# johnnypax/llm-kubernetes-minikube-sharp4dev

Hardware: AMD Instinct MI355X
Metric: RAG queries/sec (whole node) + p50 end-to-end latency, Llama-3-8B (higher is better)
Workload: dtype bf16

## Files before the change

### csrc/bindings.cpp

```cpp
#include <torch/extension.h>
#include <c10/hip/HIPStream.h>
#include "kernels.h"

namespace {

hipStream_t cur_stream() { return c10::hip::getCurrentHIPStream().stream(); }

#define CHECK_CUDA(x) TORCH_CHECK((x).is_cuda(), #x " must be a GPU tensor")
#define CHECK_BF16(x) TORCH_CHECK((x).scalar_type() == at::kBFloat16, #x " must be bfloat16")
#define CHECK_I32(x) TORCH_CHECK((x).scalar_type() == at::kInt, #x " must be int32")
#define CHECK_F32(x) TORCH_CHECK((x).scalar_type() == at::kFloat, #x " must be float32")
#define CHECK_LASTDIM(x) TORCH_CHECK((x).stride(-1) == 1, #x " must be contiguous in its last dim")
#define CHECK_CONTIG(x) TORCH_CHECK((x).is_contiguous(), #x " must be contiguous")
void check_rc(int rc, const char* name) {
  const hipError_t e = hipGetLastError();
  if (rc <= kLkAttrError && rc > kLkAttrError - 1000)
    TORCH_CHECK(false, name, ": kernel dynamic-LDS attribute refused: ", hipGetErrorString((hipError_t)(kLkAttrError - rc)));
  if (rc <= kLkLaunchError && rc > kLkLaunchError - 1000)
    TORCH_CHECK(false, name, ": kernel launch failed: ", hipGetErrorString((hipError_t)(kLkLaunchError - rc)));
  TORCH_CHECK(rc == 0, name, ": unsupported shape/config (code ", rc, ")");
  TORCH_CHECK(e == hipSuccess, name, ": kernel launch failed: ", hipGetErrorString(e));
}
#define CHECK_RC(rc, name) check_rc((rc), (name))

// ... 113 lines not shown
}

at::Tensor ws_linear(const at::Tensor& x, const at::Tensor& w, bool swiglu, int64_t bn, int64_t splits,
                     const c10::optional<at::Tensor>& out_) {
  CHECK_CUDA(x); CHECK_BF16(x); CHECK_BF16(w); CHECK_LASTDIM(x); CHECK_CONTIG(w);
  TORCH_CHECK(x.dim() == 2 && w.dim() == 2 && x.size(1) == w.size(1), "x [M,K], w [N,K]");
  check_rows16(x, "x"); check_rows16(w, "w");
  const int M = x.size(0), K = x.size(1), N = w.size(0);
  TORCH_CHECK(M >= 1 && M <= 256, "ws_linear: M must be in [1, 256]");
  const int n_out = swiglu ? N / 2 : N;
  at::Tensor out = out_ ? *out_ : at::empty({M, n_out}, x.options());
  CHECK_BF16(out); CHECK_LASTDIM(out);
  TORCH_CHECK(out.size(0) == M && out.size(1) == n_out, "out shape");
  int BN = (int)bn, S = (int)splits;
  if (BN <= 0 || S <= 0) {
    int pb = 64, ps = 1;
    lk_wsgemm_plan(M, N, K, swiglu ? 1 : 0, &pb, &ps);
    if (BN <= 0) BN = pb;
    if (S <= 0) S = ps;
  }
  at::Tensor part;
  if (S > 1) part = at::empty({(long)S * M * N}, x.options().dtype(at::kFloat));
  int rc = lk_wsgemm(bp(x), x.stride(0), bp(w), M, N, K, BN, S, swiglu ? 1 : 0, bp(out), out.stride(0),
                     S > 1 ? part.data_ptr<float>() : nullptr, cur_stream());
  CHECK_RC(rc, "ws_linear");
  return out;
}

namespace {
struct WsSplit {
  int M, N, K, BN, S;
};
WsSplit ws_split(const at::Tensor& x, const at::Tensor& w, int64_t bn, int64_t splits, const char* name) {
  CHECK_CUDA(x); CHECK_BF16(x); CHECK_BF16(w); CHECK_LASTDIM(x); CHECK_CONTIG(w);
  TORCH_CHECK(x.dim() == 2 && w.dim() == 2 && x.size(1) == w.size(1), name, ": x [M,K], w [N,K]");
  check_rows16(x, "x"); check_rows16(w, "w");
  WsSplit p{(int)x.size(0), (int)w.size(0), (int)x.size(1), (int)bn, (int)splits};
  TORCH_CHECK(p.M >= 1 && p.M <= 256, name, ": M must be in [1, 256]");
  if (p.BN <= 0 || p.S <= 0) {
    int pb = 64, ps = 1;
    lk_wsgemm_plan(p.M, p.N, p.K, 0, &pb, &ps);
    if (p.BN <= 0) p.BN = pb;
    if (p.S <= 0) p.S = ps;
  }
  TORCH_CHECK(p.S >= 2, name, ": needs a split-K plan (S >= 2)");
  return p;
}
}

at::Tensor ws_linear_rmsnorm(const at::Tensor& x, const at::Tensor& w, at::Tensor& residual,
                             const at::Tensor& norm_w, double eps, int64_t bn, int64_t splits,
                             const c10::optional<at::Tensor>& tickets) {
  const WsSplit p = ws_split(x, w, bn, splits, "ws_linear_rmsnorm");
  CHECK_CUDA(residual); CHECK_BF16(residual); CHECK_LASTDIM(residual); check_rows16(residual, "residual");
  TORCH_CHECK(residual.dim() == 2 && residual.size(0) == p.M && residual.size(1) == p.N, "residual shape");
  CHECK_BF16(norm_w); TORCH_CHECK(norm_w.numel() == p.N && norm_w.is_contiguous(), "norm weight shape");
// ... 353 lines not shown
  CHECK_RC(lk_gather_rows(bp(out), bp(x), x.stride(0), idx.data_ptr<int64_t>(), idx.numel(), x.size(1), cur_stream()),
           "gather_rows");
  return out;
}

int64_t gemm_streamk(int64_t mode) { return lk_gemm_streamk((int)mode); }

bool gemm_supported(int64_t M, int64_t N, int64_t K, int64_t epi, int64_t bn, int64_t splits, int64_t variant) {
  return gemm_shape_ok((int)M, (int)N, (int)K, (int)epi, (int)bn, (int)splits, (int)variant);
}

std::vector<int64_t> ws_plan(int64_t M, int64_t N, int64_t K, bool swiglu) {
  int bn = 64, s = 1;
  lk_wsgemm_plan((int)M, (int)N, (int)K, swiglu ? 1 : 0, &bn, &s);
  return {bn, s};
}

int64_t skinny_splits(int64_t M, int64_t N, int64_t K, bool swiglu) {
  return lk_skinny_splits((int)M, (int)N, (int)K, swiglu ? 1 : 0);
}

void activation_(at::Tensor& x, const c10::optional<at::Tensor>& bias, int64_t kind) {
  CHECK_CUDA(x); CHECK_BF16(x); CHECK_LASTDIM(x);
  TORCH_CHECK(x.dim() == 2, "x must be 2-D");
  check_rows16(x, "x");
  if (bias) { CHECK_BF16(*bias); TORCH_CHECK(bias->numel() == x.size(1), "bias shape"); }
  int rc = lk_activation(bp(x), bpo(bias), x.size(0), x.size(1), x.stride(0), (int)kind, cur_stream());
  CHECK_RC(rc, "activation");
}

// ... 460 lines not shown
           py::arg("w") = py::none(), py::arg("eps") = 1e-5)
      .def("gather", &XgmiAr::gather, "", py::arg("in"), py::arg("out"), py::arg("root") = -1)
      .def("max_bytes", &XgmiAr::max_bytes)
      .def("error", &XgmiAr::error)
      .def_readonly("bytes", &XgmiAr::bytes);
  m.doc() = "gfx950 (MI355X) HIP kernel library";
  m.def("rmsnorm", &rmsnorm, "", py::arg("x"), py::arg("w"), py::arg("eps"), py::arg("residual") = py::none(), py::arg("out") = py::none());
  m.def("layernorm", &layernorm, "", py::arg("x"), py::arg("w"), py::arg("b"), py::arg("eps"), py::arg("residual") = py::none(), py::arg("write_residual") = false);
  m.def("embed_layernorm", &embed_layernorm);
  m.def("skinny_linear", &skinny_linear, "", py::arg("x"), py::arg("w"), py::arg("swiglu") = false,
        py::arg("splits") = 0, py::arg("out") = py::none());
  m.def("skinny_splits", &skinny_splits);
  m.def("ws_linear", &ws_linear, "", py::arg("x"), py::arg("w"), py::arg("swiglu") = false, py::arg("bn") = 0,
        py::arg("splits") = 0, py::arg("out") = py::none());
  m.def("ws_plan", &ws_plan);
  m.def("gemm", &gemm, "", py::arg("x"), py::arg("w"), py::arg("bias") = py::none(), py::arg("epi") = 0,
        py::arg("bn") = 256, py::arg("out") = py::none(), py::arg("variant") = 1,
        py::arg("splits") = 1);
  m.def("gemm_fused", &gemm_fused, "", py::arg("x"), py::arg("w"), py::arg("epi"), py::arg("bn"), py::arg("out") = py::none(),
        py::arg("variant") = 2, py::arg("splits") = 1, py::arg("ss_in") = py::none(), py::arg("eps") = 1e-5,
        py::arg("resid") = py::none(), py::arg("ss_out") = py::none(), py::arg("positions") = py::none(),
        py::arg("cos_sin") = py::none(), py::arg("slots") = py::none(), py::arg("k_cache") = py::none(),
        py::arg("v_cache") = py::none(), py::arg("hq") = 0, py::arg("hkv") = 0, py::arg("hd") = 0);
  m.def("embed_rows", &embed_rows, "", py::arg("table"), py::arg("ids"), py::arg("lo") = 0, py::arg("n_local") = -1);
  m.def("embed_errors", []() { return (int64_t)lk_embed_errors(); },
        "token ids outside the (whole) embedding table seen since the last call (resets)");
  m.def("scatter_ids", &scatter_ids);
  m.def("gather_rows", &gather_rows);
  m.def("argmax_key", &argmax_key, "", py::arg("logits"), py::arg("vocab_lo") = 0);
  m.def("keys_to_ids", &keys_to_ids);
// ... 34 lines not shown
    return lk_gemv_supported((int)M, (int)N, (int)K, (int)mode) != 0;
  });
  m.def("gemv_set_wgs", [](int64_t n) { lk_gemv_set_wgs((int)n); });
  m.def("gemv_set_ksplit", [](bool on) { lk_gemv_set_ksplit(on ? 1 : 0); });
  m.def("l3_prefetch", [](const at::Tensor& t, int64_t r0, int64_t r1, int64_t wgs, at::Tensor& sink) {
    CHECK_CUDA(t); CHECK_CONTIG(t); CHECK_CUDA(sink);
    TORCH_CHECK(sink.scalar_type() == at::kInt && sink.numel() >= 1, "sink: int32 [>= 1]");
    TORCH_CHECK(t.dim() == 2 && 0 <= r0 && r0 <= r1 && r1 <= t.size(0), "rows out of range");
    const long row = t.size(1) * t.element_size();
    const char* base = reinterpret_cast<const char*>(t.data_ptr()) + r0 * row;
    CHECK_RC(lk_l3_prefetch(base, (r1 - r0) * row, (int)wgs, reinterpret_cast<unsigned*>(sink.data_ptr<int>()),
                            cur_stream()), "l3_prefetch");
  });
  m.def("ws_set_variant", [](int64_t M, int64_t N, int64_t K, bool swiglu, int64_t v) {
    CHECK_RC(lk_wsgemm_set_variant((int)M, (int)N, (int)K, swiglu ? 1 : 0, (int)v), "ws_set_variant");
  }, "weight-streaming GEMM kernel for this (M bucket, N, K, swiglu): 0 ring, 1 loader waves, -1 default",
        py::arg("M"), py::arg("N"), py::arg("K"), py::arg("swiglu"), py::arg("variant"));
  m.def("flash_prefill", &flash_prefill, "", py::arg("q"), py::arg("k"), py::arg("v"), py::arg("block_tables"), py::arg("cu_q"), py::arg("ctx_lens"), py::arg("tile_seq"), py::arg("tile_q0"), py::arg("Hq"), py::arg("Hkv"), py::arg("D"), py::arg("scale"), py::arg("causal"), py::arg("out") = py::none(), py::arg("part_o") = py::none(), py::arg("part_ml") = py::none(), py::arg("q_past") = py::none());
  m.def("knn_topk", &knn_topk, "", py::arg("corpus"), py::arg("cnorm"), py::arg("queries"), py::arg("qnorm"),
        py::arg("K"), py::arg("force_fused") = false);
  m.def("knn_merge", &knn_merge);
  m.def("pool_normalize", &pool_normalize, "", py::arg("hidden"), py::arg("cu"), py::arg("mode"), py::arg("normalize"),
        py::arg("out") = py::none());
  m.def("row_norms", &row_norms);
  m.def("select_allowed", &select_allowed, "", py::arg("logits"), py::arg("plan"), py::arg("temps") = py::none(),
        py::arg("seed") = 0, py::arg("step") = 0);
  m.def("select_tokens", &select_tokens, "", py::arg("logits"), py::arg("temps") = py::none(), py::arg("seed") = 0, py::arg("step") = 0, py::arg("out") = py::none());
  m.def("repeat_penalty_", &repeat_penalty_);
  m.def("sample", &sample, "", py::arg("logits"), py::arg("prm"), py::arg("hist"), py::arg("hist_len"),
        py::arg("seed") = 0, py::arg("out") = py::none());
}
// ... 1 lines not shown
```

### csrc/kernels.h

```cpp
#pragma once
#include <hip/hip_runtime.h>

typedef unsigned short bf16_t;

constexpr int kLkLaunchError = -1000;
constexpr int kLkAttrError = -2000;

int lk_rmsnorm(bf16_t* out, bf16_t* residual, const bf16_t* x, const bf16_t* w, long rows, int H,
               float eps, long xs, long os, long rs, hipStream_t st);
int lk_splitk_rmsnorm(bf16_t* out, bf16_t* residual, const float* part, int S, const bf16_t* w, long rows, int H,
                      float eps, long os, long rs, hipStream_t st);
int lk_layernorm(bf16_t* out, const bf16_t* x, const bf16_t* res, bf16_t* res_out, const bf16_t* w,
                 const bf16_t* b, long rows, int H, float eps, long xs, long os, long rs,
                 hipStream_t st);
int lk_embed_layernorm(bf16_t* out, const int* ids, const int* pos_ids, const int* type_ids,
                       const bf16_t* tok, const bf16_t* pos, const bf16_t* typ, const bf16_t* w,
                       const bf16_t* b, long rows, int H, float eps, hipStream_t st);

int lk_silu_mul(bf16_t* out, const bf16_t* x, long rows, int I, long xs, long os, hipStream_t st);
int lk_activation(bf16_t* x, const bf16_t* bias, long rows, int N, long xs, int kind,
                  hipStream_t st);

int lk_skinny_splits(int M, int N, int K, int swiglu);
int lk_skinny_gemm(const bf16_t* x, long ldx, const bf16_t* w, int M, int N, int K, int S, int swiglu,
// ... 16 lines not shown
                   int Hq, int Hkv, int D, bf16_t* kc, bf16_t* vc, const int* slots, int BS, int neox,
                   const float* po, const float* pml, const int* ctx, int max_splits, int split, hipStream_t st);

int lk_wsgemm_set_variant(int M, int N, int K, int swiglu, int variant);
int lk_wsgemm_part(const bf16_t* x, long ldx, const bf16_t* w, int M, int N, int K, int BN, int S, float* part,
                   hipStream_t st);
int lk_ws_rope_kv_fused(const bf16_t* x, long ldx, const bf16_t* w, int M, int K, int BN, int S, float* part,
                        int* tickets, bf16_t* qkv, long qs, const int* positions, const float* cos_sin, int Hq,
                        int Hkv, int D, bf16_t* kc, bf16_t* vc, const int* slots, int BS, int neox,
                        int write_k_inplace, hipStream_t st);
int lk_ws_rmsnorm_fused(const bf16_t* x, long ldx, const bf16_t* w, int M, int N, int K, int BN, int S, float* part,
                        int* tickets, bf16_t* out, long os, bf16_t* residual, long rs, const bf16_t* norm_w, float eps,
                        hipStream_t st);

void lk_wsgemm_set_rot(int rot_mul);

int lk_ws_scores_f32(const bf16_t* x, long ldx, const bf16_t* w, int M, long N, int K, float* out, long ldo,
                     hipStream_t st);

int lk_xgmi_ar_sig_words();
int lk_xgmi_gather(bf16_t* const* data, unsigned* const* sig, int rank, int world, int root, const void* in,
                   void* out, long nbytes, int* err, hipStream_t st);
int lk_xgmi_allreduce2(bf16_t* const* data, unsigned* const* sig, long red_off, int rank, int world,
                       const bf16_t* in, bf16_t* residual, const bf16_t* w, bf16_t* out, int T, int H, float eps,
                       int norm, int* err, hipStream_t st);
int lk_xgmi_ar_max_ranks();
int lk_xgmi_allreduce_rmsnorm(bf16_t* const* data, unsigned* const* sig, int rank, int world, const bf16_t* in,
                              bf16_t* residual, const bf16_t* w, bf16_t* out, int T, int H, float eps, int* err,
                              hipStream_t st);
int lk_xgmi_allreduce(bf16_t* const* data, unsigned* const* sig, int rank, int world, const bf16_t* in,
// ... 92 lines not shown
```

### csrc/skinny_gemm.hip

```cpp
#include <algorithm>
#include <cstdlib>
#include <map>
#include <mutex>

#include "common.h"
#include "kernels.h"

namespace {

constexpr int kSkW = 4;

LK_DEVICE float silu_f(float x) { return x / (1.f + __expf(-x)); }
LK_DEVICE float rbf(float x) { return bf2f(f2bf(x)); }

constexpr int kSysCoherent = 1 | 16;

struct WsTail {
  int kind = 0;
  int* tickets = nullptr;
  bf16_t* out = nullptr;
  long os = 0;
  const int* positions = nullptr;
  const float* cos_sin = nullptr;
  int Hq = 0, Hkv = 0, D = 0;
// ... 924 lines not shown
  if (bn96 && !swiglu) {
    int s96 = 1;
    const double o96 = plan(96, &s96);
    if (o96 > occ + 1e-9) {
      *bn_out = 96;
      *s_out = s96;
    }
  }
}

static std::mutex g_ws_var_mu;
static std::map<long, int> g_ws_var;
static long ws_var_key(int MT, int N, int K, int swiglu) {
  return (((long)MT * 1000003L + N) * 1000003L + K) * 2 + (swiglu ? 1 : 0);
}
static int ws_variant(int M, int N, int K, int swiglu) {
  static const int dflt = [] {
    const char* e = getenv("LK_WS_LOADER");
    return e ? (atoi(e) != 0) : 0;
  }();
  std::lock_guard<std::mutex> lock(g_ws_var_mu);
  auto it = g_ws_var.find(ws_var_key(ws_mt(M), N, K, swiglu));
  return it != g_ws_var.end() ? it->second : dflt;
}
int lk_wsgemm_set_variant(int M, int N, int K, int swiglu, int variant) {
  if (variant < -1 || variant > 1) return -1;
  std::lock_guard<std::mutex> lock(g_ws_var_mu);
  const long key = ws_var_key(ws_mt(M), N, K, swiglu);
  if (variant < 0) g_ws_var.erase(key);
  else g_ws_var[key] = variant;
  return 0;
}

int lk_wsgemm(const bf16_t* x, long ldx, const bf16_t* w, int M, int N, int K, int BN, int S, int swiglu,
              bf16_t* out, long ldo, float* part, hipStream_t st) {
  if (M < 1 || M > 256 || S < 1 || K % (S * 64) || (BN != 64 && BN != 128 && (BN != 96 || swiglu))) return -1;
  const int per = swiglu ? BN / 2 : BN;
  if (swiglu ? (N % 2 || (N / 2) % per) : N % BN) return -1;
  if (S > 1 && part == nullptr) return -1;
  const int I = swiglu ? N / 2 : 0;
  const int n_tiles = (swiglu ? I : N) / per;
  const int MT = ws_mt(M);
  const int ks = K / S;
  float* p = S > 1 ? part : nullptr;
  const int var = ws_variant(M, N, K, swiglu);
  const int rc = swiglu ? dispatch_ws<true>(MT, BN, x, ldx, w, M, K, ks, S, n_tiles, I, out, ldo, p, N, st,
                                            1L << 40, var)
                        : dispatch_ws<false>(MT, BN, x, ldx, w, M, K, ks, S, n_tiles, I, out, ldo, p, N, st,
                                             1L << 40, var);
  if (rc) return rc;
  if (S > 1) {
    const int n_out = swiglu ? I : N;
    const long work = (long)M * (n_out / 4);
    int grid = (int)((work + 255) / 256);
    if (grid > 2048) grid = 2048;
    if (swiglu)
      splitk_reduce_kernel<true><<<grid, 256, 0, st>>>(part, S, M, N, n_out, I, out, ldo);
    else
      splitk_reduce_kernel<false><<<grid, 256, 0, st>>>(part, S, M, N, n_out, 0, out, ldo);
  }
  LK_CHECK_LAUNCH();
  return 0;
}

// ... 50 lines not shown
    if (swiglu)
      splitk_reduce_kernel<true><<<grid, 256, 0, st>>>(part, S, M, N, n_out, I, out, ldo);
    else
      splitk_reduce_kernel<false><<<grid, 256, 0, st>>>(part, S, M, N, n_out, 0, out, ldo);
    LK_CHECK_LAUNCH();
  }
  return 0;
}

int lk_wsgemm_part(const bf16_t* x, long ldx, const bf16_t* w, int M, int N, int K, int BN, int S, float* part,
                   hipStream_t st) {
  if (M < 1 || M > 256 || S < 2 || K % (S * 64) || (BN != 64 && BN != 96 && BN != 128) || N % BN ||
      part == nullptr)
    return -1;
  const int MT = ws_mt(M);
  const int rc = dispatch_ws<false>(MT, BN, x, ldx, w, M, K, K / S, S, N / BN, 0, nullptr, 0, part, N, st,
                                    1L << 40, ws_variant(M, N, K, 0));
  LK_CHECK_LAUNCH();
  return rc;
}

int lk_ws_rope_kv_fused(const bf16_t* x, long ldx, const bf16_t* w, int M, int K, int BN, int S, float* part,
                        int* tickets, bf16_t* qkv, long qs, const int* positions, const float* cos_sin, int Hq,
                        int Hkv, int D, bf16_t* kc, bf16_t* vc, const int* slots, int BS, int neox,
                        int write_k_inplace, hipStream_t st) {
  const int N = (Hq + 2 * Hkv) * D;
  if (M < 1 || M > 256 || !(S == 2 || S == 4 || S == 8) || K % (S * 64) || BN != D || BN != 128 || !part ||
      !tickets || !qkv || qs % 8 || D % 16 || (long)S * M * N * 4 >= 0x7FFFFFF0L)
    return -1;
  WsTail tl;
  tl.kind = 1;
  tl.tickets = tickets;
// ... 90 lines not shown
```

### llm_kubernetes_minikube_sharp4dev_amd/engine/model_runner.py

```python
from __future__ import annotations

import bisect
import os
from dataclasses import dataclass, field
from typing import Optional

import numpy as np
import torch

try:
    from ..native import runtime as _nrt

    _native_rt = _nrt.load() if _nrt.available() and hasattr(_nrt.load(), "decode_rows") else None
except Exception:
    _native_rt = None

from .. import ops
from ..models import attention as _attn
from ..models.attention import AttnMeta
from ..utils.logging import get_logger

log = get_logger("engine.runner")

EXTEND_AS_DECODE = int(os.environ.get("LK_EXTEND_AS_DECODE", "16"))
# ... 101 lines not shown

            box = [dict(ops._GEMM_TABLE) if lead else None]
            dist.broadcast_object_list(box, src=tp.ranks[0] if tp.ranks else 0, group=tp.ctrl or tp.group)
            ops._GEMM_TABLE.clear()
            ops._GEMM_TABLE.update(box[0])
        return res

    @staticmethod
    def _tune_decode(model) -> dict:
        tp = getattr(model, "tp", None)
        lead = tp is None or not tp.enabled or getattr(tp, "simulated", False) or tp.rank == 0
        res = ops.tune_decode(model.decode_gemm_shapes()) if lead else {}
        if tp is not None and tp.enabled and not getattr(tp, "simulated", False):
            import torch.distributed as dist

            box = [(dict(ops._DECODE_TABLE), dict(ops._WS_VARIANTS)) if lead else None]
            dist.broadcast_object_list(box, src=tp.ranks[0] if tp.ranks else 0, group=tp.ctrl or tp.group)
            ops._DECODE_TABLE.clear()
            ops._DECODE_TABLE.update(box[0][0])
            if not lead:
                ops.apply_ws_variants(box[0][1])
        picks = {}
        for (m, n, k, sw), arm in sorted(ops._DECODE_TABLE.items()):
            picks.setdefault(f"N{n} K{k}{' swiglu' if sw else ''}", []).append(f"{m}:{arm}")
        log.info("decode GEMM routing (M bucket: kernel): %s", "; ".join(f"{k} {' '.join(v)}" for k, v in picks.items()))
        if ops._WS_VARIANTS:
            log.info("weight-streaming kernel per row tile (1 = loader waves): %s",
                     "; ".join(f"M{m} N{n} K{k}{' swiglu' if sw else ''}: {v}"
                               for (m, n, k, sw), v in sorted(ops._WS_VARIANTS.items())))
        return res

    @staticmethod
    def block_bytes(model, block_size: int) -> int:
        esz = torch.tensor([], dtype=model.dtype).element_size()
        return model.cfg.num_layers * 2 * model.hkv * block_size * model.D * esz

    @staticmethod
    def plan_num_blocks(model, block_size=16, max_model_len=8192, max_num_seqs=256, kv_cache_gb=None,
                        gpu_memory_fraction=0.85) -> int:
        bb = ModelRunner.block_bytes(model, block_size)
        if kv_cache_gb is not None:
            n = int(kv_cache_gb * (1 << 30) // bb)
        elif model.device.type == "cuda":
            free, total = torch.cuda.mem_get_info(model.device)
# ... 369 lines not shown
```

### llm_kubernetes_minikube_sharp4dev_amd/ops/__init__.py

```python
from __future__ import annotations

import logging
import math
import os
from typing import Optional, Sequence

import numpy as np
import torch

from . import reference as ref
from ._ext import available, force_reference, lib, use_hip

__all__ = [
    "rmsnorm", "layernorm", "embed_layernorm", "silu_mul", "gelu_", "relu_", "rope_kv_",
    "kv_write", "paged_decode", "flash_prefill", "prefill_tiles", "knn_topk", "knn_merge",
    "pool_normalize", "row_norms", "select_tokens", "repeat_penalty_", "sample", "linear", "linear_swiglu",
    "decode_splits", "rope_cos_sin", "argmax_key", "key_to_id", "tune_gemm", "tune_decode", "gemm", "linear_add_rmsnorm", "linear_rope_kv",
    "prefill_chain_ok", "linear_resid", "linear_qkv_fused", "linear_swiglu_scaled", "embed_rows", "scatter_ids",
    "gather_rows",
]

rope_cos_sin = ref.rope_cos_sin
DECODE_MAX_SPLIT = 2048

# ... 227 lines not shown
        return lib().sample(logits, prm, hist, hist_len, int(seed) & ((1 << 63) - 1), out)
    return ref.sample(logits, prm, hist, hist_len, seed)


def repeat_penalty_(logits, window, penalty):
    if use_hip(logits):
        lib().repeat_penalty_(logits, window, penalty)
        return logits
    return ref.repeat_penalty_(logits, window, penalty)


SKINNY_MAX_M = int(os.environ.get("LK_SKINNY_MAX_M", "0"))
LM_HEAD_SKINNY_MAX_M = 16
WS_LM_HEAD = os.environ.get("LK_WS_LM_HEAD", "0") == "1"
WS_MAX_M = int(os.environ.get("LK_WS_MAX_M", "256"))
WS_SWIGLU_MAX_M = 160


_DECODE_TABLE: dict = {}
DECODE_TUNE_MS = (32, 64, 96, 128, 160, 192, 224, 256)


def _decode_bucket(M: int) -> Optional[int]:
    for b in DECODE_TUNE_MS:
        if M <= b:
            return b
    return None


def _decode_gemm_kind(x, w, swiglu: bool) -> Optional[str]:
    if not (use_hip(x) and x.dim() == 2 and w.dim() == 2 and x.dtype == torch.bfloat16
# ... 227 lines not shown
                f()
            ts = {c: [] for c in cfgs}
            for _ in range(iters):
                for c, f in fns.items():
                    ts[c].append(once(f))
            med = {c: statistics.median(v) for c, v in ts.items()}
            key = _gemm_key(M, N, K, epi)
            _GEMM_TABLE[key] = min(med, key=med.get)
            out[key] = {f"v{c[0]}/{c[1]}/k{c[2]}": round(t, 1) for c, t in med.items()}
        del copies
    return out


WS_VARIANT_TUNE = os.environ.get("LK_WS_VARIANT_TUNE", "1") != "0"
_WS_VARIANTS: dict = {}


def apply_ws_variants(table: dict):
    _WS_VARIANTS.clear()
    _WS_VARIANTS.update(table)
    if table and available():
        L = lib()
        for (M, N, K, sw), v in table.items():
            L.ws_set_variant(M, N, K, sw, v)


def tune_decode(weights, ms: Sequence[int] = DECODE_TUNE_MS, iters: int = 5, cold_bytes: int = 640 << 20) -> dict:
    import statistics

    L = lib()
    out = {}
    for w, swiglu in weights:
        N, K = w.shape
        swiglu = bool(swiglu)
        copies = [w] + [w.clone() for _ in range(max(1, -(-cold_bytes // (N * K * 2)) - 1))]
# ... 10 lines not shown
                    for c in copies[1:] + copies[:1]:
                        fn(c)
                    b.record()
                    b.synchronize()
                    ts[k].append(a.elapsed_time(b) * 1e3 / len(copies))
            return {k: statistics.median(v) for k, v in ts.items()}

        if WS_VARIANT_TUNE and _decode_static_ok(N, K, swiglu):
            for M in [m for m in (64, 128, 192, 256) if m in ms]:
                x = torch.randn(M, K, device=w.device, dtype=torch.bfloat16)
                fns = {}
                for v in (0, 1):
                    fns[v] = (lambda c, v=v: (L.ws_set_variant(M, N, K, swiglu, v), L.ws_linear(x, c, swiglu)))
                med = timed(fns)
                best = min(med, key=med.get)
                L.ws_set_variant(M, N, K, swiglu, best)
                _WS_VARIANTS[(M, N, K, swiglu)] = best
                out[(M, N, K, swiglu, "ws_variant")] = {("ring", "loader")[v]: round(t, 1) for v, t in med.items()}
        for M in ms:
            x = torch.randn(M, K, device=w.device, dtype=torch.bfloat16)
            arms = {}
            if M <= 256 and _decode_static_ok(N, K, swiglu):
                arms["ws"] = lambda c, x=x: L.ws_linear(x, c, swiglu)
            epi = 1 if swiglu else 0
            cfg = _gemm_default(M, N, K, epi)
            if cfg is not None and L.gemm_supported(M, N, K, epi, cfg[1], cfg[2], cfg[0]):
                arms["gemm"] = lambda c, x=x, cfg=cfg: L.gemm(x, c, None, epi, cfg[1], None, cfg[0], cfg[2])
            if len(arms) < 2:
                continue
            med = timed(arms)
            _DECODE_TABLE[(M, N, K, swiglu)] = min(med, key=med.get)
            out[(M, N, K, swiglu)] = {k: round(v, 1) for k, v in med.items()}
        del copies
# ... 45 lines not shown
    if y is None:
        y = silu_mul(_library(x, w_gate_up, None, None, (True, w_gate_up.shape[0], w_gate_up.shape[1], 1)))
    return y


DECODE_FUSION = os.environ.get("LK_DECODE_FUSION", "1") != "0"
_WS_PLANS: dict = {}


def _ws_split_plan(x, w):
    if not DECODE_FUSION or _decode_gemm_kind(x, w, False) != "ws":
        return None
    key = (x.shape[0], w.shape[0], w.shape[1])
    plan = _WS_PLANS.get(key)
    if plan is None:
        plan = _WS_PLANS[key] = tuple(lib().ws_plan(*key, False))
    return plan if plan[1] in (2, 4, 8) else None


WS_FUSED_TAIL = os.environ.get("LK_WS_FUSED_TAIL", "0") == "1"
_WS_TICKETS: dict = {}


def ws_tickets(device):
    device = torch.device(device)
    key = device.index if device.index is not None else torch.cuda.current_device()
    t = _WS_TICKETS.get(key)
    if t is None:
        t = _WS_TICKETS[key] = torch.zeros(4096, dtype=torch.int32, device=device)
    return t

# ... 238 lines not shown
```

Measured before the change: 109.0.

## Add weight-streaming GEMM variant that streams weights into VGPRs, autotuned per shape

Adds a third weight-streaming decode GEMM kernel. Weight tiles are loaded with nontemporal loads straight into VGPRs across a multi-stage register pipeline, and only activations are staged through LDS via direct global-to-LDS loads, with hand-managed vmcnt waits. The tuner benchmarks this variant against the best of ring and loader for M>64 and picks it only when it measures faster. Planning and routing now go through a route function, and a static default picks the loader variant for large-M swiglu shapes. This adds heavy register pressure (one block per CU) and more code paths in exchange for less LDS traffic on weight tiles.

```diff
diff --git a/csrc/bindings.cpp b/csrc/bindings.cpp
--- a/csrc/bindings.cpp
+++ b/csrc/bindings.cpp
@@ -151,8 +151,8 @@
   TORCH_CHECK(out.size(0) == M && out.size(1) == n_out, "out shape");
   int BN = (int)bn, S = (int)splits;
   if (BN <= 0 || S <= 0) {
-    int pb = 64, ps = 1;
-    lk_wsgemm_plan(M, N, K, swiglu ? 1 : 0, &pb, &ps);
+    int pb = 64, ps = 1, pv = 0;
+    lk_wsgemm_route(M, N, K, swiglu ? 1 : 0, &pv, &pb, &ps);
     if (BN <= 0) BN = pb;
     if (S <= 0) S = ps;
   }
@@ -175,8 +175,8 @@
   WsSplit p{(int)x.size(0), (int)w.size(0), (int)x.size(1), (int)bn, (int)splits};
   TORCH_CHECK(p.M >= 1 && p.M <= 256, name, ": M must be in [1, 256]");
   if (p.BN <= 0 || p.S <= 0) {
-    int pb = 64, ps = 1;
-    lk_wsgemm_plan(p.M, p.N, p.K, 0, &pb, &ps);
+    int pb = 64, ps = 1, pv = 0;
+    lk_wsgemm_route(p.M, p.N, p.K, 0, &pv, &pb, &ps);
     if (p.BN <= 0) p.BN = pb;
     if (p.S <= 0) p.S = ps;
   }
@@ -560,6 +560,30 @@
   int bn = 64, s = 1;
   lk_wsgemm_plan((int)M, (int)N, (int)K, swiglu ? 1 : 0, &bn, &s);
   return {bn, s};
+}
+
+std::vector<int64_t> ws_plan2(int64_t M, int64_t N, int64_t K, bool swiglu) {
+  int bn = 128, s = 1;
+  lk_wsgemm2_plan((int)M, (int)N, (int)K, swiglu ? 1 : 0, &bn, &s);
+  return {bn, s};
+}
+
+std::vector<int64_t> ws_route(int64_t M, int64_t N, int64_t K, bool swiglu) {
+  int v = 0, bn = 64, s = 1;
+  lk_wsgemm_route((int)M, (int)N, (int)K, swiglu ? 1 : 0, &v, &bn, &s);
+  return {v, bn, s};
+}
+
+void ws2_part(const at::Tensor& x, const at::Tensor& w, int64_t bn, int64_t splits, at::Tensor& part) {
+  CHECK_CUDA(x); CHECK_BF16(x); CHECK_BF16(w); CHECK_LASTDIM(x); CHECK_CONTIG(w);
+  TORCH_CHECK(x.dim() == 2 && w.dim() == 2 && x.size(1) == w.size(1), "ws2_part: x [M,K], w [N,K]");
+  check_rows16(x, "x"); check_rows16(w, "w");
+  const int M = x.size(0), K = x.size(1), N = w.size(0), S = (int)splits;
+  CHECK_CUDA(part); CHECK_F32(part); CHECK_LASTDIM(part);
+  TORCH_CHECK(S >= 2 && part.dim() == 2 && part.size(0) == (long)S * M && part.size(1) == N, "ws2_part: part [S * M, N]");
+  TORCH_CHECK(lk_wsgemm2_supported(M, N, K, (int)bn, S, 0), "ws2_part: shape / plan not supported");
+  CHECK_RC(lk_wsgemm2_launch(bp(x), x.stride(0), bp(w), M, N, K, (int)bn, S, 0, nullptr, 0, part.data_ptr<float>(),
+                             part.stride(0), cur_stream()), "ws2_part");
 }
 
 int64_t skinny_splits(int64_t M, int64_t N, int64_t K, bool swiglu) {
@@ -1050,6 +1074,14 @@
   m.def("ws_linear", &ws_linear, "", py::arg("x"), py::arg("w"), py::arg("swiglu") = false, py::arg("bn") = 0,
         py::arg("splits") = 0, py::arg("out") = py::none());
   m.def("ws_plan", &ws_plan);
+  m.def("ws_plan2", &ws_plan2, "(BN, S) of weight-streaming variant 2 for this shape", py::arg("M"), py::arg("N"),
+        py::arg("K"), py::arg("swiglu") = false);
+  m.def("ws_route", &ws_route, "(variant, BN, S) this shape runs when no plan is forced", py::arg("M"), py::arg("N"),
+        py::arg("K"), py::arg("swiglu") = false);
+  m.def("ws2_supported", [](int64_t M, int64_t N, int64_t K, int64_t bn, int64_t S, bool swiglu) {
+    return lk_wsgemm2_supported((int)M, (int)N, (int)K, (int)bn, (int)S, swiglu ? 1 : 0) != 0;
+  });
+  m.def("ws2_part", &ws2_part, "", py::arg("x"), py::arg("w"), py::arg("bn"), py::arg("splits"), py::arg("part"));
   m.def("gemm", &gemm, "", py::arg("x"), py::arg("w"), py::arg("bias") = py::none(), py::arg("epi") = 0,
         py::arg("bn") = 256, py::arg("out") = py::none(), py::arg("variant") = 1,
         py::arg("splits") = 1);
@@ -1114,7 +1146,7 @@
   });
   m.def("ws_set_variant", [](int64_t M, int64_t N, int64_t K, bool swiglu, int64_t v) {
     CHECK_RC(lk_wsgemm_set_variant((int)M, (int)N, (int)K, swiglu ? 1 : 0, (int)v), "ws_set_variant");
-  }, "weight-streaming GEMM kernel for this (M bucket, N, K, swiglu): 0 ring, 1 loader waves, -1 default",
+  }, "weight-streaming GEMM kernel for this (M bucket, N, K, swiglu): 0 ring, 1 loader waves, 2 W to VGPRs, -1 default",
         py::arg("M"), py::arg("N"), py::arg("K"), py::arg("swiglu"), py::arg("variant"));
   m.def("flash_prefill", &flash_prefill, "", py::arg("q"), py::arg("k"), py::arg("v"), py::arg("block_tables"), py::arg("cu_q"), py::arg("ctx_lens"), py::arg("tile_seq"), py::arg("tile_q0"), py::arg("Hq"), py::arg("Hkv"), py::arg("D"), py::arg("scale"), py::arg("causal"), py::arg("out") = py::none(), py::arg("part_o") = py::none(), py::arg("part_ml") = py::none(), py::arg("q_past") = py::none());
   m.def("knn_topk", &knn_topk, "", py::arg("corpus"), py::arg("cnorm"), py::arg("queries"), py::arg("qnorm"),
diff --git a/csrc/kernels.h b/csrc/kernels.h
--- a/csrc/kernels.h
+++ b/csrc/kernels.h
@@ -54,6 +54,12 @@
                         hipStream_t st);
 
 void lk_wsgemm_set_rot(int rot_mul);
+
+int lk_wsgemm2_supported(int M, int N, int K, int BN, int S, int swiglu);
+int lk_wsgemm2_launch(const bf16_t* x, long ldx, const bf16_t* w, int M, int N, int K, int BN, int S, int swiglu,
+                      bf16_t* out, long ldo, float* part, long part_ld, hipStream_t st);
+void lk_wsgemm2_plan(int M, int N, int K, int swiglu, int* bn_out, int* s_out);
+void lk_wsgemm_route(int M, int N, int K, int swiglu, int* variant_out, int* bn_out, int* s_out);
 
 int lk_ws_scores_f32(const bf16_t* x, long ldx, const bf16_t* w, int M, long N, int K, float* out, long ldo,
                      hipStream_t st);
diff --git a/csrc/skinny_gemm.hip b/csrc/skinny_gemm.hip
--- a/csrc/skinny_gemm.hip
+++ b/csrc/skinny_gemm.hip
@@ -962,22 +962,59 @@
 static long ws_var_key(int MT, int N, int K, int swiglu) {
   return (((long)MT * 1000003L + N) * 1000003L + K) * 2 + (swiglu ? 1 : 0);
 }
+static int ws_env_variant() {
+  static const int v = [] {
+    const char* e = getenv("LK_WS_LOADER");
+    return e ? (atoi(e) != 0 ? 1 : 0) : -1;
+  }();
+  return v;
+}
+static int ws_static_variant(int MT, int N, int K, int swiglu) {
+  static const int on = [] {
+    const char* e = getenv("LK_WS_STATIC");
+    return e ? atoi(e) : 1;
+  }();
+  if (!on || MT < 12) return 0;
+  if (swiglu && K <= 4096) {
+    int bn = 0, s = 0;
+    lk_wsgemm_plan(16 * MT, N, K, 1, &bn, &s);
+    if (s == 1) return 1;
+  }
+  return 0;
+}
 static int ws_variant(int M, int N, int K, int swiglu) {
-  static const int dflt = [] {
-    const char* e = getenv("LK_WS_LOADER");
-    return e ? (atoi(e) != 0) : 0;
-  }();
-  std::lock_guard<std::mutex> lock(g_ws_var_mu);
-  auto it = g_ws_var.find(ws_var_key(ws_mt(M), N, K, swiglu));
-  return it != g_ws_var.end() ? it->second : dflt;
+  {
+    std::lock_guard<std::mutex> lock(g_ws_var_mu);
+    auto it = g_ws_var.find(ws_var_key(ws_mt(M), N, K, swiglu));
+    if (it != g_ws_var.end()) return it->second;
+  }
+  return ws_env_variant() >= 0 ? ws_env_variant() : ws_static_variant(ws_mt(M), N, K, swiglu);
+}
+static int ws_variant_for(int M, int N, int K, int BN, int S, int swiglu) {
+  const int var = ws_variant(M, N, K, swiglu);
+  if (var == 2 && !lk_wsgemm2_supported(M, N, K, BN, S, swiglu)) return ws_env_variant() > 0 ? 1 : 0;
+  return var;
 }
 int lk_wsgemm_set_variant(int M, int N, int K, int swiglu, int variant) {
-  if (variant < -1 || variant > 1) return -1;
+  if (variant < -1 || variant > 2) return -1;
   std::lock_guard<std::mutex> lock(g_ws_var_mu);
   const long key = ws_var_key(ws_mt(M), N, K, swiglu);
   if (variant < 0) g_ws_var.erase(key);
   else g_ws_var[key] = variant;
   return 0;
+}
+void lk_wsgemm_route(int M, int N, int K, int swiglu, int* variant_out, int* bn_out, int* s_out) {
+  int var = ws_variant(M, N, K, swiglu);
+  if (var == 2) {
+    lk_wsgemm2_plan(M, N, K, swiglu, bn_out, s_out);
+    if (lk_wsgemm2_supported(M, N, K, *bn_out, *s_out, swiglu)) {
+      *variant_out = 2;
+      return;
+    }
+    var = ws_env_variant() > 0 ? 1 : 0;
+  }
+  *variant_out = var;
+  lk_wsgemm_plan(M, N, K, swiglu, bn_out, s_out);
 }
 
 int lk_wsgemm(const bf16_t* x, long ldx, const bf16_t* w, int M, int N, int K, int BN, int S, int swiglu,
@@ -991,11 +1028,12 @@
   const int MT = ws_mt(M);
   const int ks = K / S;
   float* p = S > 1 ? part : nullptr;
-  const int var = ws_variant(M, N, K, swiglu);
-  const int rc = swiglu ? dispatch_ws<true>(MT, BN, x, ldx, w, M, K, ks, S, n_tiles, I, out, ldo, p, N, st,
-                                            1L << 40, var)
-                        : dispatch_ws<false>(MT, BN, x, ldx, w, M, K, ks, S, n_tiles, I, out, ldo, p, N, st,
-                                             1L << 40, var);
+  const int var = ws_variant_for(M, N, K, BN, S, swiglu);
+  const int rc = var == 2 ? lk_wsgemm2_launch(x, ldx, w, M, N, K, BN, S, swiglu, out, ldo, p, N, st)
+                 : swiglu ? dispatch_ws<true>(MT, BN, x, ldx, w, M, K, ks, S, n_tiles, I, out, ldo, p, N, st,
+                                              1L << 40, var)
+                          : dispatch_ws<false>(MT, BN, x, ldx, w, M, K, ks, S, n_tiles, I, out, ldo, p, N, st,
+                                               1L << 40, var);
   if (rc) return rc;
   if (S > 1) {
     const int n_out = swiglu ? I : N;
@@ -1076,8 +1114,10 @@
       part == nullptr)
     return -1;
   const int MT = ws_mt(M);
+  const int var = ws_variant_for(M, N, K, BN, S, 0);
+  if (var == 2) return lk_wsgemm2_launch(x, ldx, w, M, N, K, BN, S, 0, nullptr, 0, part, N, st);
   const int rc = dispatch_ws<false>(MT, BN, x, ldx, w, M, K, K / S, S, N / BN, 0, nullptr, 0, part, N, st,
-                                    1L << 40, ws_variant(M, N, K, 0));
+                                    1L << 40, var);
   LK_CHECK_LAUNCH();
   return rc;
 }
diff --git a/csrc/wsgemm2.hip b/csrc/wsgemm2.hip
--- /dev/null
+++ b/csrc/wsgemm2.hip
@@ -0,0 +1,326 @@
+#include <cstdlib>
+#include <type_traits>
+
+#include "common.h"
+#include "kernels.h"
+
+namespace {
+
+LK_DEVICE float ws2_silu(float x) { return x / (1.f + __expf(-x)); }
+LK_DEVICE float ws2_rbf(float x) { return bf2f(f2bf(x)); }
+
+typedef __attribute__((address_space(3))) void* ws2_lds_ptr;
+typedef const __attribute__((address_space(1))) void* ws2_gbl_ptr;
+
+LK_DEVICE int ws2_swz(int row) { return (row >> 1) & 7; }
+
+constexpr int kWs2WStages = 8;
+
+constexpr int ws2_xslots(int MT, int KB) {
+  const int n = 163840 / (KB * 16 * MT * 128);
+  return n * KB > 8 ? 8 / KB : n;
+}
+
+template <int LO, int HI>
+LK_DEVICE void ws2_wait_vm_half(int h) {
+  if constexpr (LO == HI) {
+    constexpr int N = 2 * LO;
+    static_assert(N >= 0 && N < 64, "vmcnt range");
+    __builtin_amdgcn_s_waitcnt((N & 0xF) | ((N >> 4) << 14) | (0x7 << 4) | (0xF << 8));
+  } else {
+    constexpr int MID = (LO + HI) / 2;
+    if (h <= MID) ws2_wait_vm_half<LO, MID>(h);
+    else ws2_wait_vm_half<MID + 1, HI>(h);
+  }
+}
+
+template <int MT, int NTW, bool SWIGLU, int KB>
+__global__ __launch_bounds__(256, 1) void wsgemm2_kernel(const bf16_t* __restrict__ X, long ldx,
+                                                         const bf16_t* __restrict__ W, int M, int K, int ks,
+                                                         int n_tiles, int swiglu_I, bf16_t* __restrict__ out,
+                                                         long ldo, float* __restrict__ part, long part_ld,
+                                                         int rot_mul) {
+  static_assert(!SWIGLU || NTW % 2 == 0, "a wave pairs its gate tiles with its up tiles");
+  constexpr int ROWS = 16 * MT;
+  constexpr int BN = 64 * NTW;
+  constexpr int XB = ROWS * 128;
+  constexpr int GB = KB * XB;
+  constexpr int NSX = ws2_xslots(MT, KB);
+  constexpr int P = NSX - 1;
+  constexpr int NWG = kWs2WStages / KB;
+  constexpr int LXS = ROWS / 32;
+  constexpr int LX = KB * LXS;
+  constexpr int LW = KB * NTW * 2;
+  static_assert(NSX >= 2 && LX * (P - 1) + LW * P < 64, "vmcnt range");
+  extern __shared__ __attribute__((aligned(16))) unsigned char smem[];
+
+  const int t = blockIdx.x % n_tiles, s = blockIdx.x / n_tiles;
+  const int lane = threadIdx.x & 63;
+  const int w = __builtin_amdgcn_readfirstlane(threadIdx.x >> 6);
+  const int r = lane & 15, g = lane >> 4;
+  const long kbase = (long)s * ks;
+  const int ng = ks / (64 * KB);
+  const int rot = rot_mul ? (int)(((long)t * rot_mul) % ng) : 0;
+  auto kof = [&](int gi) { return (gi + rot < ng ? gi + rot : gi + rot - ng) * (64 * KB); };
+
+  auto wcol = [&](int c) -> long {
+    if constexpr (SWIGLU) {
+      constexpr int H = NTW / 2;
+      return c < H ? (long)t * (BN / 2) + (w * H + c) * 16
+                   : (long)swiglu_I + (long)t * (BN / 2) + (w * H + c - H) * 16;
+    } else {
+      return (long)t * BN + (w * NTW + c) * 16;
+    }
+  };
+
+  const bf16_t* wp[NTW];
+#pragma unroll
+  for (int c = 0; c < NTW; ++c) wp[c] = W + (wcol(c) + r) * K + kbase + 8 * g;
+  const bf16_t* xsrc[LXS];
+  const int lrow = lane >> 3, lch = lane & 7;
+#pragma unroll
+  for (int i = 0; i < LXS; ++i) {
+    const int row = (w * LXS + i) * 8 + lrow;
+    xsrc[i] = X + (long)min(row, M - 1) * ldx + kbase + ((lch ^ ws2_swz(row)) * 8);
+  }
+
+  floatx4 acc[MT][NTW];
+#pragma unroll
+  for (int m = 0; m < MT; ++m)
+#pragma unroll
+    for (int c = 0; c < NTW; ++c) acc[m][c] = floatx4{0.f, 0.f, 0.f, 0.f};
+
+  short8 wr[NWG][KB][NTW][2];
+
+  auto load_w = [&](short8 (&f)[KB][NTW][2], int gi) {
+    const int k = kof(gi);
+#pragma unroll
+    for (int kb = 0; kb < KB; ++kb)
+#pragma unroll
+      for (int c = 0; c < NTW; ++c)
+#pragma unroll
+        for (int h = 0; h < 2; ++h)
+          f[kb][c][h] = __builtin_nontemporal_load(reinterpret_cast<const short8*>(wp[c] + k + 64 * kb + 32 * h));
+  };
+  auto issue_x = [&](int gi) {
+    unsigned char* base = smem + (gi % NSX) * GB;
+    const int k = kof(gi);
+#pragma unroll
+    for (int kb = 0; kb < KB; ++kb)
+#pragma unroll
+      for (int i = 0; i < LXS; ++i)
+        __builtin_amdgcn_global_load_lds((ws2_gbl_ptr)(xsrc[i] + k + 64 * kb),
+                                         (ws2_lds_ptr)(base + kb * XB + (w * LXS + i) * 8 * 128), 16, 0, 0);
+  };
+  auto compute = [&](const short8 (&f)[KB][NTW][2], int gi) {
+    const unsigned char* base = smem + (gi % NSX) * GB;
+    constexpr int NF = KB * 2 * MT, B = MT / 2, NB = NF / B;
+    auto xfrag = [&](int idx) -> short8 {
+      const int kb = idx / (2 * MT), h = (idx / MT) % 2, m = idx % MT;
+      const int row = 16 * m + r;
+      return *reinterpret_cast<const short8*>(base + kb * XB + row * 128 + (((4 * h + g) ^ ws2_swz(row)) << 4));
+    };
+    short8 a[2][B];
+#pragma unroll
+    for (int i = 0; i < B; ++i) a[0][i] = xfrag(i);
+#pragma unroll
+    for (int b = 0; b < NB; ++b) {
+#pragma unroll
+      for (int i = 0; i < B; ++i) {
+        if (i == 1 && b + 1 < NB) {
+#pragma unroll
+          for (int n = 0; n < B; ++n) a[(b + 1) % 2][n] = xfrag((b + 1) * B + n);
+        }
+        const int idx = b * B + i;
+        const int kb = idx / (2 * MT), h = (idx / MT) % 2, m = idx % MT;
+#pragma unroll
+        for (int c = 0; c < NTW; ++c)
+          acc[m][c] = __builtin_amdgcn_mfma_f32_16x16x32_bf16(f[kb][c][h], a[b % 2][i], acc[m][c], 0, 0, 0);
+      }
+    }
+    __builtin_amdgcn_sched_group_barrier(0x100, B, 0);
+#pragma unroll
+    for (int b = 0; b < NB; ++b) {
+      __builtin_amdgcn_sched_group_barrier(0x008, NTW, 0);
+      if (b + 1 < NB) __builtin_amdgcn_sched_group_barrier(0x100, B, 0);
+      __builtin_amdgcn_sched_group_barrier(0x008, (B - 1) * NTW, 0);
+    }
+  };
+
+  const int nx = max(0, ng - P), nw = max(0, ng - NWG);
+  auto pending = [&](int gi) -> int {
+    const int before = min(P, ng) * LX + LX * min(gi, nx) + LW * min(gi, nw);
+    const int through = gi < P ? (gi + 1) * LX : P * LX + LX * (gi - P + 1) + LW * min(gi - P, nw);
+    return before - through;
+  };
+
+  auto stage = [&](auto full, short8 (&f)[KB][NTW][2], int gi) {
+    constexpr bool FULL = decltype(full)::value;
+    __builtin_amdgcn_sched_barrier(0);
+    constexpr int STEADY = LX * (P - 1) + LW * P;
+    static_assert(LX % 2 == 0 && LW % 2 == 0, "even counts");
+    if (FULL && gi >= P) ws2_wait_vm_half<STEADY / 2, STEADY / 2>(STEADY / 2);
+    else ws2_wait_vm_half<0, STEADY / 2>(min(max(pending(gi), 0), STEADY) / 2);
+    __builtin_amdgcn_s_barrier();
+    __builtin_amdgcn_sched_barrier(0);
+    if (FULL || gi + P < ng) issue_x(gi + P);
+    __builtin_amdgcn_sched_barrier(0);
+    compute(f, gi);
+    if (FULL || gi + NWG < ng) load_w(f, gi + NWG);
+  };
+
+#pragma unroll
+  for (int p = 0; p < NWG; ++p)
+    if (p < ng) load_w(wr[p], p);
+#pragma unroll
+  for (int p = 0; p < P; ++p)
+    if (p < ng) issue_x(p);
+
+  int gi = 0;
+  for (; gi + 2 * NWG <= ng; gi += NWG) {
+#pragma unroll
+    for (int j = 0; j < NWG; ++j) stage(std::true_type{}, wr[j], gi + j);
+  }
+  for (; gi < ng; gi += NWG) {
+#pragma unroll
+    for (int j = 0; j < NWG; ++j)
+      if (gi + j < ng) stage(std::false_type{}, wr[j], gi + j);
+  }
+
+  const bool split = part != nullptr;
+  const bool part_vec = split && part_ld % 4 == 0 && reinterpret_cast<uintptr_t>(part) % 16 == 0;
+  const bool out_vec = ldo % 4 == 0 && reinterpret_cast<uintptr_t>(out) % 8 == 0;
+#pragma unroll
+  for (int m = 0; m < MT; ++m) {
+    const int row = 16 * m + r;
+    if (row >= M) continue;
+    if (SWIGLU && !split) {
+#pragma unroll
+      for (int c = 0; c < NTW / 2; ++c) {
+        float y[4];
+#pragma unroll
+        for (int i = 0; i < 4; ++i)
+          y[i] = ws2_rbf(ws2_silu(ws2_rbf(acc[m][c][i]))) * ws2_rbf(acc[m][c + NTW / 2][i]);
+        bf16_t* dst = out + (long)row * ldo + wcol(c) + 4 * g;
+        if (out_vec) {
+          uint2 pk;
+          pk.x = pack_bf2(y[0], y[1]);
+          pk.y = pack_bf2(y[2], y[3]);
+          *reinterpret_cast<uint2*>(dst) = pk;
+        } else {
+#pragma unroll
+          for (int i = 0; i < 4; ++i) dst[i] = f2bf(y[i]);
+        }
+      }
+    } else if (split) {
+#pragma unroll
+      for (int c = 0; c < NTW; ++c) {
+        float* dst = part + ((long)s * M + row) * part_ld + wcol(c) + 4 * g;
+        if (part_vec) {
+          *reinterpret_cast<floatx4*>(dst) = acc[m][c];
+        } else {
+#pragma unroll
+          for (int i = 0; i < 4; ++i) dst[i] = acc[m][c][i];
+        }
+      }
+    } else {
+#pragma unroll
+      for (int c = 0; c < NTW; ++c) {
+        bf16_t* dst = out + (long)row * ldo + wcol(c) + 4 * g;
+        if (out_vec) {
+          uint2 pk;
+          pk.x = pack_bf2(acc[m][c][0], acc[m][c][1]);
+          pk.y = pack_bf2(acc[m][c][2], acc[m][c][3]);
+          *reinterpret_cast<uint2*>(dst) = pk;
+        } else {
+#pragma unroll
+          for (int i = 0; i < 4; ++i) dst[i] = f2bf(acc[m][c][i]);
+        }
+      }
+    }
+  }
+}
+
+int ws2_kb() {
+  static const int kb = [] {
+    const char* e = getenv("LK_WS2_KB");
+    const int v = e ? atoi(e) : 2;
+    return v == 1 ? 1 : 2;
+  }();
+  return kb;
+}
+
+template <int MT, int NTW, bool SWIGLU, int KB>
+void launch_ws2(const bf16_t* x, long ldx, const bf16_t* w, int M, int K, int ks, int S, int n_tiles, int I,
+                bf16_t* out, long ldo, float* part, long part_ld, hipStream_t st) {
+  constexpr size_t lds = (size_t)ws2_xslots(MT, KB) * KB * 16 * MT * 128;
+  static_assert(lds <= 163840, "LDS");
+  LK_SET_MAX_LDS((wsgemm2_kernel<MT, NTW, SWIGLU, KB>), (int)lds);
+  const int rot_mul = S == 1 ? 5 : 0;
+  wsgemm2_kernel<MT, NTW, SWIGLU, KB><<<n_tiles * S, 256, lds, st>>>(x, ldx, w, M, K, ks, n_tiles, I, out, ldo, part,
+                                                                   part_ld, rot_mul);
+}
+
+template <int MT>
+int dispatch_ws2(int NTW, bool swiglu, int KB, const bf16_t* x, long ldx, const bf16_t* w, int M, int K, int ks, int S,
+                 int n_tiles, int I, bf16_t* out, long ldo, float* part, long part_ld, hipStream_t st) {
+#define LK_WS2(ntw, sw, kb)                                                                        \
+  if (NTW == ntw && swiglu == sw && KB == kb) {                                                    \
+    launch_ws2<MT, ntw, sw, kb>(x, ldx, w, M, K, ks, S, n_tiles, I, out, ldo, part, part_ld, st); \
+    return 0;                                                                                      \
+  }
+  LK_WS2(1, false, 1) LK_WS2(1, false, 2) LK_WS2(2, false, 1) LK_WS2(2, false, 2) LK_WS2(2, true, 1) LK_WS2(2, true, 2)
+#undef LK_WS2
+  return -2;
+}
+
+}
+
+int lk_wsgemm2_supported(int M, int N, int K, int BN, int S, int swiglu) {
+  if (M <= 64 || M > 256 || S < 1 || K < 64 || K % (S * 64)) return 0;
+  if (BN != 128 && (BN != 64 || swiglu)) return 0;
+  if (swiglu ? (N % 2 || (N / 2) % (BN / 2)) : N % BN) return 0;
+  return 1;
+}
+
+void lk_wsgemm2_plan(int M, int N, int K, int swiglu, int* bn_out, int* s_out) {
+  int best_bn = 128, best_s = 1, best_blocks = -1;
+  for (int bn : {128, 64}) {
+    for (int S : {1, 2, 4, 8}) {
+      if (!lk_wsgemm2_supported(M > 64 ? M : 65, N, K, bn, S, swiglu) || (S > 1 && K / S < 512)) continue;
+      const int blocks = (swiglu ? N / bn : N / bn) * S;
+      if (blocks > 256 && best_blocks >= 0) continue;
+      const bool better = best_blocks < 0 || (best_blocks > 256 && blocks <= 256) ||
+                          (blocks <= 256 && (blocks > best_blocks || (blocks == best_blocks && S < best_s))) ||
+                          (best_blocks > 256 && blocks < best_blocks);
+      if (better) {
+        best_bn = bn;
+        best_s = S;
+        best_blocks = blocks;
+      }
+    }
+  }
+  *bn_out = best_bn;
+  *s_out = best_s;
+}
+
+int lk_wsgemm2_launch(const bf16_t* x, long ldx, const bf16_t* w, int M, int N, int K, int BN, int S, int swiglu,
+                      bf16_t* out, long ldo, float* part, long part_ld, hipStream_t st) {
+  if (!lk_wsgemm2_supported(M, N, K, BN, S, swiglu)) return -1;
+  if (S > 1 ? part == nullptr || part_ld < N : out == nullptr) return -1;
+  const int I = swiglu ? N / 2 : 0;
+  const int n_tiles = (swiglu ? I : N) / (swiglu ? BN / 2 : BN);
+  const int ks = K / S;
+  const int KB = (ks / 64) % 2 == 0 ? ws2_kb() : 1;
+  float* p = S > 1 ? part : nullptr;
+  const int MT = M <= 128 ? 8 : M <= 192 ? 12 : 16;
+  int rc;
+  switch (MT) {
+    case 8: rc = dispatch_ws2<8>(BN / 64, swiglu != 0, KB, x, ldx, w, M, K, ks, S, n_tiles, I, out, ldo, p, part_ld, st); break;
+    case 12: rc = dispatch_ws2<12>(BN / 64, swiglu != 0, KB, x, ldx, w, M, K, ks, S, n_tiles, I, out, ldo, p, part_ld, st); break;
+    default: rc = dispatch_ws2<16>(BN / 64, swiglu != 0, KB, x, ldx, w, M, K, ks, S, n_tiles, I, out, ldo, p, part_ld, st); break;
+  }
+  if (rc) return rc;
+  LK_CHECK_LAUNCH();
+  return 0;
+}
diff --git a/llm_kubernetes_minikube_sharp4dev_amd/engine/model_runner.py b/llm_kubernetes_minikube_sharp4dev_amd/engine/model_runner.py
--- a/llm_kubernetes_minikube_sharp4dev_amd/engine/model_runner.py
+++ b/llm_kubernetes_minikube_sharp4dev_amd/engine/model_runner.py
@@ -139,7 +139,7 @@
         if tp is not None and tp.enabled and not getattr(tp, "simulated", False):
             import torch.distributed as dist
 
-            box = [(dict(ops._DECODE_TABLE), dict(ops._WS_VARIANTS)) if lead else None]
+            box = [(dict(ops._DECODE_TABLE), ops.ws_variant_table()) if lead else None]
             dist.broadcast_object_list(box, src=tp.ranks[0] if tp.ranks else 0, group=tp.ctrl or tp.group)
             ops._DECODE_TABLE.clear()
             ops._DECODE_TABLE.update(box[0][0])
@@ -150,9 +150,9 @@
             picks.setdefault(f"N{n} K{k}{' swiglu' if sw else ''}", []).append(f"{m}:{arm}")
         log.info("decode GEMM routing (M bucket: kernel): %s", "; ".join(f"{k} {' '.join(v)}" for k, v in picks.items()))
         if ops._WS_VARIANTS:
-            log.info("weight-streaming kernel per row tile (1 = loader waves): %s",
+            log.info("weight-streaming kernel per row tile (1 = loader waves, 2 = W to VGPRs): %s",
                      "; ".join(f"M{m} N{n} K{k}{' swiglu' if sw else ''}: {v}"
-                               for (m, n, k, sw), v in sorted(ops._WS_VARIANTS.items())))
+                               for (m, n, k, sw), v in sorted(ops.ws_variant_table().items())))
         return res
 
     @staticmethod
diff --git a/llm_kubernetes_minikube_sharp4dev_amd/ops/__init__.py b/llm_kubernetes_minikube_sharp4dev_amd/ops/__init__.py
--- a/llm_kubernetes_minikube_sharp4dev_amd/ops/__init__.py
+++ b/llm_kubernetes_minikube_sharp4dev_amd/ops/__init__.py
@@ -265,7 +265,7 @@
 LM_HEAD_SKINNY_MAX_M = 16
 WS_LM_HEAD = os.environ.get("LK_WS_LM_HEAD", "0") == "1"
 WS_MAX_M = int(os.environ.get("LK_WS_MAX_M", "256"))
-WS_SWIGLU_MAX_M = 160
+WS_SWIGLU_MAX_M = int(os.environ.get("LK_WS_SWIGLU_MAX_M", "160"))
 
 
 _DECODE_TABLE: dict = {}
@@ -523,11 +523,22 @@
 
 WS_VARIANT_TUNE = os.environ.get("LK_WS_VARIANT_TUNE", "1") != "0"
 _WS_VARIANTS: dict = {}
+_WS_VARIANT_NAMES = ("ring", "loader", "vgpr")
+
+
+_WS_V2: set = set()
+
+
+def ws_variant_table() -> dict:
+    return {k: (2 if k in _WS_V2 else v) for k, v in _WS_VARIANTS.items()}
 
 
 def apply_ws_variants(table: dict):
     _WS_VARIANTS.clear()
-    _WS_VARIANTS.update(table)
+    _WS_VARIANTS.update({k: (0 if v == 2 else v) for k, v in table.items()})
+    _WS_V2.clear()
+    _WS_V2.update(k for k, v in table.items() if v == 2)
+    _WS_PLANS.clear()
     if table and available():
         L = lib()
         for (M, N, K, sw), v in table.items():
@@ -568,9 +579,19 @@
                     fns[v] = (lambda c, v=v: (L.ws_set_variant(M, N, K, swiglu, v), L.ws_linear(x, c, swiglu)))
                 med = timed(fns)
                 best = min(med, key=med.get)
+                _WS_VARIANTS[(M, N, K, swiglu)] = best
+                _WS_V2.discard((M, N, K, swiglu))
+                out[(M, N, K, swiglu, "ws_variant")] = {_WS_VARIANT_NAMES[v]: round(t, 1) for v, t in med.items()}
+                if M > 64 and L.ws2_supported(M, N, K, *L.ws_plan2(M, N, K, swiglu), swiglu):
+                    med2 = timed({v: fns.get(v) or (lambda c, v=v: (L.ws_set_variant(M, N, K, swiglu, v),
+                                                                   L.ws_linear(x, c, swiglu))) for v in (best, 2)})
+                    out[(M, N, K, swiglu, "ws_variant", "vgpr")] = {_WS_VARIANT_NAMES[v]: round(t, 1)
+                                                                   for v, t in med2.items()}
+                    if med2[2] < med2[best]:
+                        _WS_V2.add((M, N, K, swiglu))
+                        best = 2
                 L.ws_set_variant(M, N, K, swiglu, best)
-                _WS_VARIANTS[(M, N, K, swiglu)] = best
-                out[(M, N, K, swiglu, "ws_variant")] = {("ring", "loader")[v]: round(t, 1) for v, t in med.items()}
+                _WS_PLANS.clear()
         for M in ms:
             x = torch.randn(M, K, device=w.device, dtype=torch.bfloat16)
             arms = {}
@@ -646,7 +667,7 @@
     key = (x.shape[0], w.shape[0], w.shape[1])
     plan = _WS_PLANS.get(key)
     if plan is None:
-        plan = _WS_PLANS[key] = tuple(lib().ws_plan(*key, False))
+        plan = _WS_PLANS[key] = tuple(lib().ws_route(*key, False))[1:]
     return plan if plan[1] in (2, 4, 8) else None
 
 
```

Result: no change. 109.1, median of 2 (+0.1%).
